# scvae/scvae

Hardware: AMD Instinct MI355X
Metric: cells/sec training (68k-PBMC NB-VAE) (higher is better)
Workload: dtype f32 (bf16x9-exact heads); 1 GPU; 68k-PBMC-shaped synthetic counts 68579x32738 (~5% nonzero, device CSR), negative binomial VAE hidden 100-100 latent 25 batch-norm, Adam lr 1e-4; global_batch=4096, parallelism=dp1

## Files before the change

scvae_amd/csrc/decoder_fused3.hip:

```cpp
#include <type_traits>

#include "common.hpp"
#include "kernels.hpp"
#include "likelihood.hpp"

namespace scvae {

typedef float f32x16 __attribute__((ext_vector_type(16)));
typedef float f32x4m __attribute__((ext_vector_type(4)));
typedef __bf16 bf16x8 __attribute__((ext_vector_type(8)));
typedef short s16x4 __attribute__((ext_vector_type(4)));
typedef short s16x8 __attribute__((ext_vector_type(8)));
typedef unsigned u32x4 __attribute__((ext_vector_type(4)));
typedef unsigned u32x2 __attribute__((ext_vector_type(2)));
typedef float f32x2 __attribute__((ext_vector_type(2)));
typedef float f32x4u __attribute__((ext_vector_type(4), aligned(4)));

#ifndef D3_PIN_LOADS
#define D3_PIN_LOADS 1
#endif
#ifndef D3_AHEAD
#define D3_AHEAD 1
#endif
constexpr int D3_NB = D3_AHEAD + 1;
__device__ __forceinline__ void d3_pin_loads() {
  if (D3_PIN_LOADS) __builtin_amdgcn_sched_barrier(0x7C6);
}

constexpr int D3_THREADS = 512;
constexpr int D3_BM = 64;
constexpr int D3_KP = 128;
__host__ __device__ constexpr int d3_bn(int P) { return P >= 3 ? 32 : 64; }
__host__ __device__ constexpr int d3_rowb(int P) { return 2 * d3_bn(P) + 16; }

__host__ __device__ inline int d3_hp1(int H) { return (H + 1 + 15) / 16 * 16; }

int decoder_fused3_strip_genes(int P) { return d3_bn(P); }
size_t decoder_fused3_lds_bytes(int P, int H) {
  return (size_t)P * 3 * d3_hp1(H) * d3_rowb(P) + (size_t)P * 3 * D3_BM * d3_rowb(P) +
         2 * D3_BM * sizeof(float);
}
bool decoder_fused3_supported(int P, int H) {
  return P <= 3 && H >= 2 && H <= 126 && decoder_fused3_lds_bytes(P, H) <= 160 * 1024;
}
__host__ __device__ inline int d3_kp(int H) { return H + 1 <= D3_KP ? D3_KP : (H + 1 + 31) / 32 * 32; }
__host__ __device__ inline size_t d3_set_elems(int Rpad, int KP = D3_KP) {
  return (size_t)2 * 3 * Rpad * KP;
}
size_t decoder_fused3_workspace_floats(int rows, int H) {
  const size_t rpad = (size_t)(rows + D3_BM - 1) / D3_BM * D3_BM;
  const int kp = d3_kp(H);
  if (kp > D3_KP) return d3_set_elems((int)rpad, kp) * sizeof(uint16_t) / sizeof(float) + 64;
  return 3 * d3_set_elems((int)rpad) * sizeof(uint16_t) / sizeof(float) + 3 * rpad * 4 + 64;
}

typedef __bf16 bf16x2 __attribute__((ext_vector_type(2)));
typedef float f32x2v __attribute__((ext_vector_type(2)));
__device__ __forceinline__ unsigned cvt_pk_bf16(float lo, float hi) {
  return __builtin_bit_cast(unsigned, __builtin_convertvector(f32x2v{lo, hi}, bf16x2));
}
__device__ __forceinline__ void split3_rn(float x, unsigned& b1, unsigned& b2, unsigned& b3) {
  b1 = cvt_pk_bf16(0.f, x) & 0xFFFF0000u;
  const float r1 = x - __uint_as_float(b1);
  b2 = cvt_pk_bf16(0.f, r1) & 0xFFFF0000u;
  b3 = __float_as_uint(r1 - __uint_as_float(b2));
}
__device__ __forceinline__ unsigned pack_hi16(unsigned lo, unsigned hi) {
  return __builtin_amdgcn_perm(hi, lo, 0x07060302u);
}
__device__ __forceinline__ void split3_rn_pair(float x0, float x1, unsigned& p1, unsigned& p2,
                                               unsigned& p3) {
  p1 = cvt_pk_bf16(x0, x1);
  float r0 = x0 - __uint_as_float(p1 << 16), r1 = x1 - __uint_as_float(p1 & 0xFFFF0000u);
  p2 = cvt_pk_bf16(r0, r1);
  r0 -= __uint_as_float(p2 << 16);
  r1 -= __uint_as_float(p2 & 0xFFFF0000u);
  p3 = pack_hi16(__float_as_uint(r0), __float_as_uint(r1));
}

__global__ __launch_bounds__(256) void split3_hidden_kernel(const float* __restrict__ d, int R,
                                                            int H, int Rpad, int KP,
                                                            uint16_t* __restrict__ dA,
                                                            uint16_t* __restrict__ dT,
                                                            u32x4* __restrict__ zero,
                                                            size_t zero16) {
  const int slot = blockIdx.x * 256 + threadIdx.x;
  for (size_t i = (size_t)(blockIdx.y * gridDim.x + blockIdx.x) * 256 + threadIdx.x; i < zero16;
       i += (size_t)gridDim.x * gridDim.y * 256)
    zero[i] = u32x4{0u, 0u, 0u, 0u};
  if (slot >= Rpad * (KP / 8)) return;
  const int ksp = KP / 32;
  const int lane = slot & 63, frag = slot >> 6;
  const int nb = Rpad / 16;
  unsigned t1[8], t2[8], t3[8];
  auto value = [&](int r, int k) {
    if (r >= R) return 0.f;
    return k < H ? d[(size_t)r * H + k] : (k == H ? 1.f : 0.f);
  };
  if (blockIdx.y == 0) {
    const int rb = frag / ksp, ks = frag % ksp;
    const int row = 16 * rb + (lane & 15), k0 = 32 * ks + 8 * (lane >> 4);
#pragma unroll
    for (int e = 0; e < 8; ++e) split3_rn(value(row, k0 + e), t1[e], t2[e], t3[e]);
  } else {
    const int ht = frag / nb, kg = frag % nb;
    const int h = 32 * ht + (lane & 31), r0 = 16 * kg + 8 * (lane >> 5);
#pragma unroll
    for (int e = 0; e < 8; ++e) split3_rn(value(r0 + e, h), t1[e], t2[e], t3[e]);
  }
  auto pack = [](const unsigned* t) {
    u32x4 v;
    v.x = pack_hi16(t[0], t[1]); v.y = pack_hi16(t[2], t[3]);
    v.z = pack_hi16(t[4], t[5]); v.w = pack_hi16(t[6], t[7]);
    return v;
  };
  const size_t plane = (size_t)KP * Rpad;
  uint16_t* dst = (blockIdx.y == 0 ? dA : dT) + (size_t)slot * 8;
  *reinterpret_cast<u32x4*>(dst) = pack(t1);
  *reinterpret_cast<u32x4*>(dst + plane) = pack(t2);
  *reinterpret_cast<u32x4*>(dst + 2 * plane) = pack(t3);
}

__device__ __forceinline__ bf16x8 lds_b128(const char* p) {
  return __builtin_bit_cast(bf16x8, *reinterpret_cast<const u32x4*>(p));
}
__device__ __forceinline__ s16x4 lds_tr(const char* p) {
  return __builtin_amdgcn_ds_read_tr16_b64_v4i16(
      (__attribute__((address_space(3))) s16x4*)(p));
}
template <int ROWB>
__device__ __forceinline__ bf16x8 lds_tr8(const char* p) {
  const s16x4 lo = lds_tr(p), hi = lds_tr(p + 4 * ROWB);
  return __builtin_bit_cast(bf16x8, __builtin_shufflevector(lo, hi, 0, 1, 2, 3, 4, 5, 6, 7));
}
__device__ __forceinline__ bf16x8 global_b128(const uint16_t* p) {
  return __builtin_bit_cast(bf16x8, *reinterpret_cast<const u32x4*>(p));
}

struct IndexMasks3 { unsigned long long m[3]; };
__device__ __forceinline__ IndexMasks3 index_masks3(int idx) {
  IndexMasks3 k;
#pragma unroll
  for (int b = 0; b < 3; ++b) k.m[b] = __builtin_amdgcn_ballot_w64((idx >> b) & 1);
  return k;
}
__device__ __forceinline__ float cnd3(float lo, float hi, unsigned long long mask) {
  float r;
  asm("v_cndmask_b32_e64 %0, %1, %2, %3" : "=v"(r) : "v"(lo), "v"(hi), "s"(mask));
  return r;
}
__device__ __forceinline__ float select_n(const float (&v)[8], const IndexMasks3& k) {
  float a[4], b[2];
#pragma unroll
  for (int i = 0; i < 4; ++i) a[i] = cnd3(v[2 * i], v[2 * i + 1], k.m[0]);
#pragma unroll
  for (int i = 0; i < 2; ++i) b[i] = cnd3(a[2 * i], a[2 * i + 1], k.m[1]);
  return cnd3(b[0], b[1], k.m[2]);
}
__device__ __forceinline__ float select_n(const float (&v)[4], const IndexMasks3& k) {
  return cnd3(cnd3(v[0], v[1], k.m[0]), cnd3(v[2], v[3], k.m[0]), k.m[1]);
}

template <int KIND, int KS1, bool U16, bool TRAIN, bool DROP, int CP>
__global__ __launch_bounds__(D3_THREADS) void decoder_head3_kernel(
    const uint16_t* __restrict__ dA, const uint16_t* __restrict__ dT, int R, int Rpad, int H,
    HeadParams hp, int F, Targets tg, int B, const float* __restrict__ gw, int inline_lgamma,
    float* __restrict__ ll_part, float* __restrict__ dd_part,
    const uint32_t* __restrict__ drop_bits, float inv_keep, CpRows cp) {
  constexpr bool IDX = false;
  const int64_t* const trows = nullptr;
#include "decoder_head3_body.inc"
}
template <int KIND, int KS1, bool TRAIN>
__global__ __launch_bounds__(D3_THREADS) void decoder_head3_rows_kernel(
    const uint16_t* __restrict__ dA, const uint16_t* __restrict__ dT, int R, int Rpad, int H,
    HeadParams hp, int F, Targets tg, int B, const float* __restrict__ gw, int inline_lgamma,
    float* __restrict__ ll_part, float* __restrict__ dd_part,
    const int64_t* __restrict__ trows) {
  constexpr bool U16 = true, DROP = false, IDX = true;
  constexpr int CP = 0;
  const uint32_t* const drop_bits = nullptr;
  const float inv_keep = 1.f;
  const CpRows cp = CpRows();
#include "decoder_head3_body.inc"
}


constexpr int D4_BM = 32;

#ifndef D4_COMPACT
#define D4_COMPACT 1
#endif
__host__ __device__ constexpr bool d4_compact(int ks1) { return D4_COMPACT && ks1 <= 4; }
__host__ __device__ constexpr int d4_threads(int npw) { return (npw + 4) * 64; }
size_t decoder_fused4_lds_bytes(int P, int H, int npw, int bn = 0) {
  const int rowb = 2 * (bn ? bn : d3_bn(P)) + 16;
  return (size_t)P * 3 * d3_hp1(H) * rowb + (size_t)2 * P * 3 * D4_BM * rowb +
         (size_t)2 * (npw / 2) * 4 * D4_BM * sizeof(float) +
         (d4_compact((H + 1 + 31) / 32) ? npw * 512 : 0);
}

#ifndef D4_PROF
#define D4_PROF 0
#endif
#ifndef D4_PRIO_PRODUCER
#define D4_PRIO_PRODUCER 1
#endif
#ifndef D4_PRIO_CONSUMER
#define D4_PRIO_CONSUMER 0
#endif
#if D4_PROF
__device__ unsigned long long d4_prof[12 * 8];
#define D4_STAMP(k)                                            \
  do {                                                         \
    __builtin_amdgcn_sched_barrier(0);                         \
    const unsigned long long t_ = __builtin_amdgcn_s_memtime(); \
    pacc[k] += t_ - plast;                                     \
    plast = t_;                                                \
    __builtin_amdgcn_sched_barrier(0);                         \
  } while (0)
#define D4_PROF_BEGIN unsigned long long pacc[8] = {0, 0, 0, 0, 0, 0, 0, 0}, plast = __builtin_amdgcn_s_memtime()
#define D4_PROF_END                                                                  \
  do {                                                                               \
    if (blockIdx.x == 0 && lane == 0)                                                \
      for (int k_ = 0; k_ < 8; ++k_) d4_prof[w * 8 + k_] = pacc[k_];                 \
  } while (0)
#else
#define D4_STAMP(k) do {} while (0)
#define D4_PROF_BEGIN do {} while (0)
#define D4_PROF_END do {} while (0)
#endif

#ifndef D4_G1_EIGHT
#define D4_G1_EIGHT 0
#endif
template <int KIND, int KS1, bool U16, int NPW, int BN_ = 0, bool DBP = false,
          int G1 = (NPW == 4 ? 1 : D4_G1_EIGHT), int TERMS = 9, bool FWD = false>
__global__ __launch_bounds__(d4_threads(NPW)) void decoder_head4_kernel(
    const uint16_t* __restrict__ dA, const uint16_t* __restrict__ dT, int R, int Rpad, int H,
    HeadParams hp, int F, Targets tg, int B, const float* __restrict__ gw, int inline_lgamma,
    float* __restrict__ ll_part, float* __restrict__ dd_part, int dd_atomic, int rg_tiles,
    float* __restrict__ rg_slab) {
  constexpr bool IDX = false;
  const int64_t* const trows = nullptr;
#include "decoder_head4_body.inc"
}
template <int KIND, int KS1, int NPW, int BN_, bool DBP, int G1, bool FWD>
__global__ __launch_bounds__(d4_threads(NPW)) void decoder_head4_rows_kernel(
    const uint16_t* __restrict__ dA, const uint16_t* __restrict__ dT, int R, int Rpad, int H,
    HeadParams hp, int F, Targets tg, int B, const float* __restrict__ gw, int inline_lgamma,
    float* __restrict__ ll_part, float* __restrict__ dd_part, int dd_atomic, int rg_tiles,
    float* __restrict__ rg_slab, const int64_t* __restrict__ trows) {
  constexpr bool U16 = true, IDX = true;
  constexpr int TERMS = 9;
#include "decoder_head4_body.inc"
}

#if D4_PROF
extern "C" int scvae_d4_prof_dump(unsigned long long* out) {
  return (int)hipMemcpyFromSymbol(out, HIP_SYMBOL(d4_prof), sizeof(unsigned long long) * 96);
}
#endif

static int d3_schedule_env() {
  static const int v = [] {
    const char* e = getenv("SCVAE_D3_SCHEDULE");
    return (e && (e[0] == '3' || e[0] == '4')) ? e[0] - '0' : 0;
  }();
  return v;
}
static int d4_producers_env() {
  static const int v = [] {
    const char* e = getenv("SCVAE_D4_PRODUCERS");
    return (e && (e[0] == '4' || e[0] == '8')) ? e[0] - '0' : 0;
  }();
  return v;
}
struct D4Config { int bn, npw, ks1; size_t lds; bool ok; bool dbp; };
static D4Config d4_config(int P, int H) {
  D4Config c;
  c.ks1 = (H + 1 + 31) / 32;
  c.bn = d3_bn(P);
  c.npw = P >= 3 ? 4 : (d4_producers_env() ? d4_producers_env() : (P == 1 ? 4 : 8));
  c.lds = decoder_fused4_lds_bytes(P, H, c.npw, c.bn);
  if (c.lds > 160 * 1024 && c.bn == 64 && P == 2) {
    c.bn = 32; c.npw = 4;
    c.lds = decoder_fused4_lds_bytes(P, H, c.npw, c.bn);
  }
  if (c.ks1 > 4 && c.npw == 8) {
    c.npw = 4;
    c.lds = decoder_fused4_lds_bytes(P, H, c.npw, c.bn);
  }
  c.dbp = H >= 128 && H % 32 == 0;
  c.ok = P >= 1 && P <= 3 && H >= 2 && c.ks1 <= (c.dbp ? 9 : 8) && c.lds <= 160 * 1024;
  return c;
}
bool decoder_fused4_supported(int P, int H) { return d4_config(P, H).ok; }
static int d3_schedule(int P, int H, int rows) {
  if (!decoder_fused3_supported(P, H)) return 4;
  if (!decoder_fused4_supported(P, H)) return 3;
  return d3_schedule_env() ? d3_schedule_env() : (rows <= 128 ? 3 : 4);
}
int d4_strip_genes(int P, int H) { return d4_config(P, H).bn; }
int decoder_fused3_train_strip_genes(int P, int H, int rows, bool drop, int cp_pass) {
  if (!drop && cp_pass == 0 && d3_schedule(P, H, rows) == 4) return d4_config(P, H).bn;
  return d3_bn(P);
}

bool decoder_fused3_dd_atomics(int kind, int H, int rows, bool drop, int cp_pass, int dd_mode) {
  const int P = likelihood_heads(kind);
  return (dd_mode & 1) && !(dd_mode & 4) && !drop && cp_pass == 0 && d3_schedule(P, H, rows) == 4;
}

int decoder_fused3_train_kernel_name(int kind, int H, int rows, bool u16, char* out, size_t n,
                                     int terms) {
  const int P = likelihood_heads(kind);
  if (d3_schedule(P, H, rows) == 4) {
    const D4Config c = d4_config(P, H);
    const bool six = terms == 6 && c.ks1 <= 4 && c.bn == d3_bn(P) && !c.dbp;
    return snprintf(out, n, "decoder_head4_kernel<%d, %d, %s, %d, %d, %s, %d, %d, false>", kind, c.ks1,
                    u16 ? "true" : "false", c.npw, c.bn == d3_bn(P) ? 0 : c.bn,
                    c.dbp ? "true" : "false", c.npw == 4 ? 1 : D4_G1_EIGHT, six ? 6 : 9);
  }
  return snprintf(out, n, "decoder_head3_kernel<%d, %d, %s, true, false, 0>", kind,
                  (d3_hp1(H) + 31) / 32, u16 ? "true" : "false");
}

constexpr int D4_MAX_ROW_GROUPS = 4;
size_t decoder_fused3_rg_slab_floats(int H, int F) {
  return (size_t)(D4_MAX_ROW_GROUPS - 1) * 3 * (size_t)(H + 1) * F + 64;
}
static int d4_cu_count() {
  static thread_local int cached_device = -1, cached = 0;
  int device = 0;
  if (hipGetDevice(&device) != hipSuccess) return 256;
  if (device != cached_device) {
    hipDeviceProp_t prop;
    cached = hipGetDeviceProperties(&prop, device) == hipSuccess ? prop.multiProcessorCount : 256;
    cached_device = device;
  }
  return cached > 0 ? cached : 256;
}
static int d4_row_groups(int strips, int rows) {
  static const int forced = [] {
    const char* e = getenv("SCVAE_D4_ROW_GROUPS");
    return e ? atoi(e) : 0;
  }();
  const int tiles = (rows + D4_BM - 1) / D4_BM;
  int most = tiles / 8;
  if (most > D4_MAX_ROW_GROUPS) most = D4_MAX_ROW_GROUPS;
  if (most < 1) most = 1;
  if (forced >= 1) return forced < most ? forced : most;
  const int cus = d4_cu_count();
  int best = 1;
  double best_score = 0.0;
  for (int n = 1; n <= most; ++n) {
    const long wgs = (long)strips * n;
    const long rounds = (wgs + cus - 1) / cus;
    const double score = (double)wgs / (double)(rounds * cus) - 0.04 * (n - 1);
    if (score > best_score + 1e-9) { best = n; best_score = score; }
  }
  return best;
}
__global__ __launch_bounds__(256) void d4_rg_combine_kernel(HeadParams hp, int P, int H, int F,
                                                            const float* __restrict__ slab,
                                                            int groups) {
  const int jh = blockIdx.y;
  const int j = jh / (H + 1), h = jh % (H + 1);
  float* dst = h < H ? hp.dW[j] + (size_t)h * F : hp.db[j];
  const size_t gstride = (size_t)P * (H + 1) * F;
  const float* src = slab + ((size_t)j * (H + 1) + h) * F;
  for (int c = blockIdx.x * blockDim.x + threadIdx.x; c < F; c += gridDim.x * blockDim.x) {
    float v = dst[c];
    for (int g = 0; g < groups; ++g) v += src[(size_t)g * gstride + c];
    dst[c] = v;
  }
}

struct D4Launch {
  hipStream_t s; const uint16_t* dA; const uint16_t* dT; int rows, Rpad, H; HeadParams hp; int F;
  Targets t; int B; const float* gw; int inline_lgamma; float* ll_part; float* dd_part;
  int dd_atomic; int strips; size_t lds; int terms; int row_groups; float* rg_slab;
  bool fwd = false;
  const int64_t* trows = nullptr;
};
template <int KIND, int KS1, int NPW, int BN_, bool DBP = false, int TERMS = 9>
static int d4_launch_one(const D4Launch& a) {
  constexpr int G1 = NPW == 4 ? 1 : D4_G1_EIGHT;
  if constexpr (TERMS == 9 && KS1 <= 4 && BN_ == 0 && !DBP) {
    if (a.terms == 6) return d4_launch_one<KIND, KS1, NPW, BN_, DBP, 6>(a);
  }
  const int tiles = (a.rows + D4_BM - 1) / D4_BM;
  const int rg_tiles = (tiles + a.row_groups - 1) / a.row_groups;
  const int groups = (tiles + rg_tiles - 1) / rg_tiles;
  if (a.trows) {
    if constexpr (TERMS == 9) {
      if (!a.t.u16 || a.terms != 9) {
        set_error("decoder_head4_kernel: a row index goes with uint16 targets and nine terms");
        return -1;
      }
      auto rfn = a.fwd ? decoder_head4_rows_kernel<KIND, KS1, NPW, BN_, DBP, G1, true>
                       : decoder_head4_rows_kernel<KIND, KS1, NPW, BN_, DBP, G1, false>;
      SCVAE_HIP(max_dynamic_lds(reinterpret_cast<const void*>(rfn), (int)a.lds));
      hipLaunchKernelGGL(rfn, dim3(a.strips, groups), dim3(d4_threads(NPW)), a.lds, a.s, a.dA,
                         a.dT, a.rows, a.Rpad, a.H, a.hp, a.F, a.t, a.B, a.gw, a.inline_lgamma,
                         a.ll_part, a.dd_part, a.fwd ? 0 : a.dd_atomic, rg_tiles,
                         a.fwd ? nullptr : a.rg_slab, a.trows);
      if (!a.fwd && groups > 1) {
        constexpr int P = likelihood_heads(KIND);
        hipLaunchKernelGGL(d4_rg_combine_kernel, dim3((a.F + 1023) / 1024, P * (a.H + 1)),
                           dim3(256), 0, a.s, a.hp, P, a.H, a.F, a.rg_slab, groups - 1);
      }
      return 0;
    }
  }
  if constexpr (TERMS == 9) {
    if (a.fwd) {
      auto ffn = a.t.u16 ? decoder_head4_kernel<KIND, KS1, true, NPW, BN_, DBP, G1, 9, true>
                         : decoder_head4_kernel<KIND, KS1, false, NPW, BN_, DBP, G1, 9, true>;
      SCVAE_HIP(max_dynamic_lds(reinterpret_cast<const void*>(ffn), (int)a.lds));
      hipLaunchKernelGGL(ffn, dim3(a.strips, groups), dim3(d4_threads(NPW)), a.lds, a.s, a.dA,
                         a.dT, a.rows, a.Rpad, a.H, a.hp, a.F, a.t, a.B, a.gw, a.inline_lgamma,
                         a.ll_part, a.dd_part, 0, rg_tiles, nullptr);
      return 0;
    }
  }
  auto kfn = a.t.u16 ? decoder_head4_kernel<KIND, KS1, true, NPW, BN_, DBP, G1, TERMS>
                     : decoder_head4_kernel<KIND, KS1, false, NPW, BN_, DBP, G1, TERMS>;
  SCVAE_HIP(max_dynamic_lds(reinterpret_cast<const void*>(kfn), (int)a.lds));
  hipLaunchKernelGGL(kfn, dim3(a.strips, groups), dim3(d4_threads(NPW)), a.lds, a.s, a.dA, a.dT,
                     a.rows, a.Rpad, a.H, a.hp, a.F, a.t, a.B, a.gw, a.inline_lgamma, a.ll_part,
                     a.dd_part, a.dd_atomic, rg_tiles, a.rg_slab);
  if (groups > 1) {
    constexpr int P = likelihood_heads(KIND);
    hipLaunchKernelGGL(d4_rg_combine_kernel, dim3((a.F + 1023) / 1024, P * (a.H + 1)), dim3(256), 0,
                       a.s, a.hp, P, a.H, a.F, a.rg_slab, groups - 1);
  }
  return 0;
}
template <int KIND, int KS1>
static int d4_launch_steps(const D4Launch& a, const D4Config& c) {
  constexpr int P = likelihood_heads(KIND);
  if constexpr (KS1 >= 5) {
    if (c.dbp) {
      if constexpr (P == 1) return d4_launch_one<KIND, KS1, 4, 0, true>(a);
      else if constexpr (P == 2) return d4_launch_one<KIND, KS1, 4, 32, true>(a);
      else if constexpr (KS1 == 5) return d4_launch_one<KIND, KS1, 4, 0, true>(a);
    }
  }
  if constexpr (KS1 == 9) {
    set_error("decoder_head4_kernel: nine contraction steps only at H = 256");
    return -1;
  } else if constexpr (P == 1) {
    if constexpr (KS1 <= 4) { if (c.npw == 8) return d4_launch_one<KIND, KS1, 8, 0>(a); }
    return d4_launch_one<KIND, KS1, 4, 0>(a);
  } else if constexpr (P == 2) {
    if constexpr (KS1 <= 4) {
      if (c.bn == 64) return c.npw == 8 ? d4_launch_one<KIND, KS1, 8, 0>(a)
                                        : d4_launch_one<KIND, KS1, 4, 0>(a);
    }
    if constexpr (KS1 >= 4) return d4_launch_one<KIND, KS1, 4, 32>(a);
    set_error("decoder_head4_kernel: no instantiation for %d steps on %d-gene strips", KS1, c.bn);
    return -1;
  } else {
    if constexpr (KS1 <= 5) return d4_launch_one<KIND, KS1, 4, 0>(a);
    set_error("decoder_head4_kernel: three heads beyond H = 159");
    return -1;
  }
}
template <int KIND>
static int d4_launch_kind(const D4Launch& a, const D4Config& c) {
  switch (c.ks1) {
    case 1: return d4_launch_steps<KIND, 1>(a, c);
    case 2: return d4_launch_steps<KIND, 2>(a, c);
    case 3: return d4_launch_steps<KIND, 3>(a, c);
    case 4: return d4_launch_steps<KIND, 4>(a, c);
    case 5: return d4_launch_steps<KIND, 5>(a, c);
    case 6: return d4_launch_steps<KIND, 6>(a, c);
    case 7: return d4_launch_steps<KIND, 7>(a, c);
    case 8: return d4_launch_steps<KIND, 8>(a, c);
    case 9: return d4_launch_steps<KIND, 9>(a, c);
    default: set_error("decoder_head4_kernel: %d contraction steps", c.ks1); return -1;
  }
}

int decoder_fused3_launch(hipStream_t s, bool train, int kind, const float* d, int rows, int H,
                          HeadParams hp, int F, Targets t, int B, const float* gw,
                          int inline_lgamma, float* ll_part, float* dd_part, float* planes,
                          const HeadDropout* drop, int cp_pass, const CpRows* cp, int dd_mode,
                          float* rg_slab, const int64_t* t_rows) {
  const int P = likelihood_heads(kind);
  SCVAE_ARG(!t_rows || (t.u16 && kind <= LK_ZINB && !drop && cp_pass == 0 && !(dd_mode & 6)));
  const bool wide = !decoder_fused3_supported(P, H) ||
                    (!train && cp_pass == 0 &&
                     (P > 2 || !decoder_fused_supported(H) || (dd_mode & 8)));
  SCVAE_ARG(!(dd_mode & 4) || (train && !wide && !drop && cp_pass == 0));
  SCVAE_ARG((hp.gene_stride == 0 && t.shift == 0.f) || (dd_mode & 4));
  SCVAE_ARG(planes && (!wide || (!drop && cp_pass == 0 && decoder_fused4_supported(P, H))));
  SCVAE_ARG(train || !drop);
  SCVAE_ARG((kind == LK_CPOISSON) == (cp_pass >= 1 && cp_pass <= 3 && cp && cp->count_sum));
  SCVAE_ARG(cp_pass == 0 || ((cp_pass == 3) == train && !drop));
  const CpRows cpr = cp ? *cp : CpRows();
  const int Rpad = (rows + D3_BM - 1) / D3_BM * D3_BM;
  const int KP = d3_kp(H);
  uint16_t* dA = reinterpret_cast<uint16_t*>(planes);
  uint16_t* dT = dA + (size_t)3 * Rpad * KP;
  uint32_t* bits = reinterpret_cast<uint32_t*>(dA + 3 * d3_set_elems(Rpad));
  const bool head4_train = train && !(dd_mode & 4) && !drop && cp_pass == 0 &&
                           d3_schedule(P, H, rows) == 4;
  const size_t acc_bytes = (size_t)8 * H * rows * sizeof(float);
  const bool clear_here = head4_train && (dd_mode & 1) && (acc_bytes & 15) == 0 &&
                          (reinterpret_cast<uintptr_t>(dd_part) & 15) == 0;
  for (int j = 0; j < (drop ? P : 1); ++j) {
    hipLaunchKernelGGL(split3_hidden_kernel, dim3((Rpad * (KP / 8) + 255) / 256, train ? 2 : 1),
                       dim3(256), 0, s, drop ? drop->d[j] : d, rows, H, Rpad, KP,
                       dA + j * d3_set_elems(Rpad), dT + j * d3_set_elems(Rpad),
                       clear_here ? reinterpret_cast<u32x4*>(dd_part) : nullptr,
                       clear_here ? acc_bytes / 16 : (size_t)0);
    SCVAE_LAUNCH_CHECK("split3_hidden_kernel");
    if (drop) {
      const int rc = dropout_mask_words(s, bits + (size_t)j * Rpad * 4, rows, Rpad, H, drop->keep,
                                        drop->seed, drop->site[j], drop->map);
      if (rc) return rc;
    }
  }
  const float inv_keep = drop ? 1.f / drop->keep : 1.f;
  const size_t lds = decoder_fused3_lds_bytes(P, H);
  const int strips = (F + d3_bn(P) - 1) / d3_bn(P);
  const int ks1 = (d3_hp1(H) + 31) / 32;
#define SCVAE_D3KC(K_, KS_, T_, D_, C_)                                                          \
  do {                                                                                            \
    auto kfn = t.u16 ? decoder_head3_kernel<K_, KS_, true, T_, D_, C_>                            \
                     : decoder_head3_kernel<K_, KS_, false, T_, D_, C_>;                          \
    SCVAE_HIP(max_dynamic_lds(reinterpret_cast<const void*>(kfn), \
                                  (int)lds));         \
    hipLaunchKernelGGL(kfn, dim3(strips), dim3(D3_THREADS), lds, s, dA, dT, rows, Rpad, H, hp, F, \
                       t, B, gw, inline_lgamma, ll_part, dd_part, bits, inv_keep, cpr);           \
  } while (0)
#define SCVAE_D3K(K_, KS_, T_, D_) SCVAE_D3KC(K_, KS_, T_, D_, 0)
#define SCVAE_D3RK(K_, KS_, T_)                                                                   \
  do {                                                                                            \
    auto kfn = decoder_head3_rows_kernel<K_, KS_, T_>;                                            \
    SCVAE_HIP(max_dynamic_lds(reinterpret_cast<const void*>(kfn), (int)lds));                     \
    hipLaunchKernelGGL(kfn, dim3(strips), dim3(D3_THREADS), lds, s, dA, dT, rows, Rpad, H, hp, F, \
                       t, B, gw, inline_lgamma, ll_part, dd_part, t_rows);                        \
  } while (0)
#define SCVAE_D3R(K_, T_)                                                                         \
  switch (ks1) {                                                                                  \
    case 1: SCVAE_D3RK(K_, 1, T_); break;                                                         \
    case 2: SCVAE_D3RK(K_, 2, T_); break;                                                         \
    case 3: SCVAE_D3RK(K_, 3, T_); break;                                                         \
    default: SCVAE_D3RK(K_, 4, T_); break;                                                        \
  }
#define SCVAE_D3C(T_, C_)                                                                         \
  switch (ks1) {                                                                                  \
    case 1: SCVAE_D3KC(LK_CPOISSON, 1, T_, false, C_); break;                                     \
    case 2: SCVAE_D3KC(LK_CPOISSON, 2, T_, false, C_); break;                                     \
    case 3: SCVAE_D3KC(LK_CPOISSON, 3, T_, false, C_); break;                                     \
    default: SCVAE_D3KC(LK_CPOISSON, 4, T_, false, C_); break;                                    \
  }
#define SCVAE_D3(K_, T_, D_)                                                                      \
  switch (ks1) {                                                                                  \
    case 1: SCVAE_D3K(K_, 1, T_, D_); break;                                                      \
    case 2: SCVAE_D3K(K_, 2, T_, D_); break;                                                      \
    case 3: SCVAE_D3K(K_, 3, T_, D_); break;                                                      \
    default: SCVAE_D3K(K_, 4, T_, D_); break;                                                     \
  }
  if (train && decoder_fused_probe(0)) SCVAE_HIP(hipEventRecord(decoder_fused_probe(0), s));
  if (cp_pass == 1) {
    SCVAE_D3C(false, 1);
  } else if (cp_pass == 2) {
    SCVAE_D3C(false, 2);
  } else if (cp_pass == 3) {
    SCVAE_D3C(true, 3);
  } else if (train && drop) {
    switch (kind) {
      case LK_POISSON: SCVAE_D3(LK_POISSON, true, true); break;
      case LK_NB: SCVAE_D3(LK_NB, true, true); break;
      case LK_ZIP: SCVAE_D3(LK_ZIP, true, true); break;
      case LK_ZINB: SCVAE_D3(LK_ZINB, true, true); break;
      case LK_BERNOULLI: SCVAE_D3(LK_BERNOULLI, true, true); break;
      default: set_error("decoder_head3_kernel: likelihood kind %d", kind); return -1;
    }
  } else if ((train && !(dd_mode & 4) && d3_schedule(P, H, rows) == 4) || (!train && wide)) {
    const D4Config c = d4_config(P, H);
    D4Launch a{s, dA, dT, rows, Rpad, H, hp, F, t, B, gw, inline_lgamma, ll_part, dd_part,
               (dd_mode & 1) ? 1 : 0, (F + c.bn - 1) / c.bn, c.lds, (dd_mode & 2) ? 6 : 9, 1,
               rg_slab};
    a.fwd = !train;
    a.trows = t_rows;
    if (a.fwd) { a.dd_atomic = 0; a.terms = 9; }
    if (rg_slab || a.fwd) a.row_groups = d4_row_groups(a.strips, rows);
    if (a.dd_atomic && !clear_here)
      SCVAE_HIP(hipMemsetAsync(dd_part, 0, (size_t)8 * H * rows * sizeof(float), s));
    int rc;
    switch (kind) {
      case LK_POISSON: rc = d4_launch_kind<LK_POISSON>(a, c); break;
      case LK_NB: rc = d4_launch_kind<LK_NB>(a, c); break;
      case LK_ZIP: rc = d4_launch_kind<LK_ZIP>(a, c); break;
      case LK_ZINB: rc = d4_launch_kind<LK_ZINB>(a, c); break;
      case LK_BERNOULLI: rc = d4_launch_kind<LK_BERNOULLI>(a, c); break;
      default: set_error("decoder_head4_kernel: likelihood kind %d", kind); return -1;
    }
    if (rc) return rc;
  } else if (t_rows && train) {
    switch (kind) {
      case LK_POISSON: SCVAE_D3R(LK_POISSON, true); break;
      case LK_NB: SCVAE_D3R(LK_NB, true); break;
      case LK_ZIP: SCVAE_D3R(LK_ZIP, true); break;
      default: SCVAE_D3R(LK_ZINB, true); break;
    }
  } else if (t_rows) {
    switch (kind) {
      case LK_POISSON: SCVAE_D3R(LK_POISSON, false); break;
      case LK_NB: SCVAE_D3R(LK_NB, false); break;
      case LK_ZIP: SCVAE_D3R(LK_ZIP, false); break;
      default: set_error("decoder_head3_kernel (forward): likelihood kind %d", kind); return -1;
    }
  } else if (train) {
    switch (kind) {
      case LK_POISSON: SCVAE_D3(LK_POISSON, true, false); break;
      case LK_NB: SCVAE_D3(LK_NB, true, false); break;
      case LK_ZIP: SCVAE_D3(LK_ZIP, true, false); break;
      case LK_ZINB: SCVAE_D3(LK_ZINB, true, false); break;
      case LK_BERNOULLI: SCVAE_D3(LK_BERNOULLI, true, false); break;
      case LK_CAT2: SCVAE_D3(LK_CAT2, true, false); break;
      case LK_CAT3: SCVAE_D3(LK_CAT3, true, false); break;
      default: set_error("decoder_head3_kernel: likelihood kind %d", kind); return -1;
    }
  } else {
    switch (kind) {
      case LK_POISSON: SCVAE_D3(LK_POISSON, false, false); break;
      case LK_NB: SCVAE_D3(LK_NB, false, false); break;
      case LK_ZIP: SCVAE_D3(LK_ZIP, false, false); break;
      case LK_BERNOULLI: SCVAE_D3(LK_BERNOULLI, false, false); break;
      default: set_error("decoder_head3_kernel (forward): likelihood kind %d", kind); return -1;
    }
  }
#undef SCVAE_D3
#undef SCVAE_D3R
#undef SCVAE_D3RK
#undef SCVAE_D3C
#undef SCVAE_D3KC
#undef SCVAE_D3K
  SCVAE_LAUNCH_CHECK("decoder_head3_kernel");
  if (train && decoder_fused_probe(1)) SCVAE_HIP(hipEventRecord(decoder_fused_probe(1), s));
  return 0;
}

}
```

scvae_amd/csrc/decoder_head4_body.inc:

```
  using Traits = LikelihoodTraits<KIND>;
  constexpr int P = Traits::P;
  constexpr int NT = d4_threads(NPW);
  constexpr int BN = BN_ ? BN_ : d3_bn(P), ROWB = 2 * BN + 16;
  constexpr int NT2 = DBP ? KS1 - 1 : KS1;
  constexpr int NHT = (NT2 + 3) / 4;
  static_assert(!DBP || (NPW == 4 && KS1 >= 2), "DBP: four producers");
  constexpr int DF = KS1 < 4 ? KS1 : 4;
  constexpr int GPLANE = D4_BM * ROWB;
  constexpr int GBUF = P * 3 * GPLANE;
  constexpr int NGP = NPW / 2;
  constexpr int NSB = BN / (16 * NGP);
  static_assert(NSB >= 1 && NSB * 16 * NGP == BN, "producer waves tile the strip");
  constexpr int NE = 4 * NSB;
  constexpr int KS3 = BN / 16;
  constexpr int NGT = BN / 32;
  constexpr int LLN = NGP * 4 * D4_BM;
  extern __shared__ __attribute__((aligned(16))) char smem[];
  const int HP1 = d3_hp1(H);
  const int WPLANE = HP1 * ROWB;
  char* Wl = smem;
  char* Gl = smem + (size_t)P * 3 * WPLANE;
  float* llbuf = reinterpret_cast<float*>(Gl + 2 * GBUF);
  const int tid = threadIdx.x, lane = tid & 63;
  const int w = __builtin_amdgcn_readfirstlane(tid >> 6);
  const int q = lane >> 4, i16 = lane & 15, li = lane & 31, kh = lane >> 5;
  const int c0 = blockIdx.x * BN;
  const int dbg = D4_PROF ? inline_lgamma >> 8 : 0;
  inline_lgamma &= 0xFF;

  constexpr int HSTEP = NT / BN;
  constexpr int NV = (32 * KS1 + HSTEP - 1) / HSTEP;
  {
    const int g = tid & (BN - 1), h0 = tid / BN;
    const bool col_ok = c0 + g < F;
    const int gc = min(c0 + g, F - 1);
    float v[P][NV];
#pragma unroll
    for (int j = 0; j < P; ++j) {
      const float* wj = hp.W[j] + gc;
      const float* bj = hp.b[j] + gc;
#pragma unroll
      for (int u = 0; u < NV; ++u) {
        const int h = min(h0 + u * HSTEP, H);
        const float* src = h < H ? wj + (size_t)h * F : bj;
        v[j][u] = *src;
      }
    }
    {
      const int n16 = (int)(((size_t)P * 3 * WPLANE + 2 * GBUF + 2 * LLN * 4) / 16);
      u32x4* z = reinterpret_cast<u32x4*>(smem);
      for (int i = tid; i < n16; i += NT) z[i] = u32x4{0u, 0u, 0u, 0u};
    }
    __syncthreads();
#pragma unroll
    for (int j = 0; j < P; ++j)
#pragma unroll
      for (int u = 0; u < NV; ++u) {
        const int h = h0 + u * HSTEP;
        if (h <= H) {
          unsigned b1, b2, b3;
          split3_rn(col_ok ? v[j][u] : 0.f, b1, b2, b3);
          char* dst = Wl + (size_t)(j * 3) * WPLANE + h * ROWB + 2 * g;
          *reinterpret_cast<uint16_t*>(dst) = (uint16_t)(b1 >> 16);
          *reinterpret_cast<uint16_t*>(dst + WPLANE) = (uint16_t)(b2 >> 16);
          *reinterpret_cast<uint16_t*>(dst + 2 * WPLANE) = (uint16_t)(b3 >> 16);
        }
      }
  }
  __syncthreads();

  const int tile0 = blockIdx.y * rg_tiles;
  const int n_tiles = min((R + D4_BM - 1) / D4_BM, tile0 + rg_tiles);
  const int mfirst = tile0 * D4_BM;
  auto grad_row = [&](int j, int h) -> float* {
    if (blockIdx.y == 0) return h < H ? hp.dW[j] + (size_t)h * F : hp.db[j];
    return rg_slab + (((size_t)(blockIdx.y - 1) * P + j) * (H + 1) + h) * F;
  };
  const int KP = d3_kp(H), ksp = KP / 32;
  const size_t dplane = (size_t)Rpad * KP;
  const int nb16 = Rpad / 16;

  if (w < NPW) {
    __builtin_amdgcn_s_setprio(D4_PRIO_PRODUCER);
    const int gp = w % NGP, rq = w / NGP;
    const int gbase = 16 * NSB * gp;
    const int trw = (8 * q + (i16 >> 2)) * ROWB + 2 * (gbase + 4 * (i16 & 3));
    const int gst = (16 * rq + i16) * ROWB + 2 * (gbase + 4 * q);
    struct TileIn { f32x4m t[NSB]; float up0; };
    size_t tidx = 0;
    auto load_i = [&](int m0) -> size_t {
      const int rc = min(m0 + 16 * rq + i16, R - 1);
      return (size_t)trows[R == B ? rc : rc % B];
    };
    if (IDX) tidx = load_i(mfirst);
    auto load_t = [&](int m0) {
      TileIn in;
      const int row = m0 + 16 * rq + i16;
      const bool rok = row < R;
      in.up0 = (rok && !FWD) ? gw[row] : 0.f;
      const int rc = rok ? row : R - 1;
      const int cell = R == B ? rc : rc % B;
      const size_t trow = (IDX ? tidx : (size_t)cell) * tg.ld;
#pragma unroll
      for (int sb = 0; sb < NSB; ++sb) {
        const int c = c0 + gbase + 16 * sb + 4 * q;
        f32x4m v = {0.f, 0.f, 0.f, 0.f};
        if (U16) {
          const uint16_t* tp = static_cast<const uint16_t*>(tg.p) + trow + c;
          const u32x2 u = *reinterpret_cast<const u32x2*>(tp);
          v.x = __uint_as_float(u.x); v.y = __uint_as_float(u.y);
        } else {
          const float* tp = static_cast<const float*>(tg.p) + trow + c;
          if (c + 3 < F) {
            const f32x4u u = *reinterpret_cast<const f32x4u*>(tp);
            v.x = u.x; v.y = u.y; v.z = u.z; v.w = u.w;
          } else {
            v.x = (c < F) ? tp[0] : 0.f;
            v.y = (c + 1 < F) ? tp[1] : 0.f;
            v.z = (c + 2 < F) ? tp[2] : 0.f;
          }
        }
        in.t[sb] = v;
      }
      return in;
    };
    bf16x8 dfr[DF][3];
    auto load_dk = [&](int m0, int ks, bf16x8 (&dst)[3]) {
      const uint16_t* dbase = dA + ((size_t)(m0 / 16 + rq) * ksp + ks) * 512 + lane * 8;
#pragma unroll
      for (int pl = 0; pl < 3; ++pl) dst[pl] = global_b128(dbase + pl * dplane);
    };
    auto load_d = [&](int m0) {
#pragma unroll
      for (int ks = 0; ks < DF; ++ks) load_dk(m0, ks, dfr[ks]);
    };
    f32x4m acc1[P][NSB];
    auto gemm1 = [&](int mt) {
#pragma unroll
      for (int j = 0; j < P; ++j)
#pragma unroll
        for (int sb = 0; sb < NSB; ++sb) acc1[j][sb] = f32x4m{0.f, 0.f, 0.f, 0.f};
      bf16x8 afr[2][P][NSB][3];
      auto load_w = [&](int ks, bf16x8 (&dst)[P][NSB][3]) {
#pragma unroll
        for (int j = 0; j < P; ++j)
#pragma unroll
          for (int sb = 0; sb < NSB; ++sb)
#pragma unroll
            for (int pl = 0; pl < 3; ++pl)
              dst[j][sb][pl] = lds_tr8<ROWB>(Wl + (size_t)(j * 3 + pl) * WPLANE + trw + 32 * sb +
                                             32 * ks * ROWB);
      };
      load_w(0, afr[0]);
#pragma unroll
      for (int ks = 0; ks < KS1; ++ks) {
        if (ks + 1 < KS1) load_w(ks + 1, afr[(ks + 1) & 1]);
#pragma unroll
        for (int a = 2; a >= 0; --a)
#pragma unroll
          for (int b = 2; b >= 0; --b)
#pragma unroll
            for (int j = 0; j < P; ++j)
#pragma unroll
              for (int sb = 0; sb < NSB; ++sb)
                if (TERMS == 9 || a + b < 3) acc1[j][sb] = __builtin_amdgcn_mfma_f32_16x16x32_bf16(
                    afr[ks & 1][j][sb][a], dfr[ks % DF][b], acc1[j][sb], 0, 0, 0);
        if (ks + DF < KS1) {
          load_dk(mt, ks + DF, dfr[ks % DF]);
          d3_pin_loads();
        }
      }
    };
    float dbacc[P][NE];
#pragma unroll
    for (int j = 0; j < P; ++j)
#pragma unroll
      for (int e = 0; e < NE; ++e) dbacc[j][e] = 0.f;
    TileIn nxt = load_t(mfirst);
    if (IDX) tidx = load_i(min(mfirst + D4_BM, Rpad - D4_BM));
    load_d(mfirst);
    const bool g1last = G1 == 1 || (G1 == 2 && w >= NPW / 2);
    if (g1last) {
      gemm1(mfirst);
      load_d(min(mfirst + D4_BM, Rpad - D4_BM));
      d3_pin_loads();
    }
    D4_PROF_BEGIN;
    for (int tile = tile0; tile < n_tiles; ++tile) {
      const int m0 = tile * D4_BM;
      if (dbg & 2) { lds_barrier(); continue; }
      const TileIn cur = nxt;
      const float up = cur.up0;
      char* Gb = Gl + ((tile - tile0) & 1) * GBUF;
      float* lb = llbuf + ((tile - tile0) & 1) * LLN;
      if (!g1last) gemm1(m0);
      {
        nxt = load_t(min(m0 + D4_BM, Rpad - D4_BM));
        if (IDX) tidx = load_i(min(m0 + 2 * D4_BM, Rpad - D4_BM));
        if (!g1last) load_d(min(m0 + D4_BM, Rpad - D4_BM));
        d3_pin_loads();
      }
      float G[P][NE], tval[NE];
      float lsum = 0.f;
      unsigned nz = 0;
#pragma unroll
      for (int sb = 0; sb < NSB; ++sb) {
        if (U16) {
          const unsigned v0 = __float_as_uint(cur.t[sb][0]), v1 = __float_as_uint(cur.t[sb][1]);
          tval[4 * sb] = (float)(v0 & 0xFFFFu); tval[4 * sb + 1] = (float)(v0 >> 16);
          tval[4 * sb + 2] = (float)(v1 & 0xFFFFu); tval[4 * sb + 3] = (float)(v1 >> 16);
        } else {
#pragma unroll
          for (int e = 0; e < 4; ++e) tval[4 * sb + e] = cur.t[sb][e];
        }
#pragma unroll
        for (int e = 0; e < 4; ++e) {
          float a[P], g[P], lp, r, rgate;
#pragma unroll
          for (int j = 0; j < P; ++j) a[j] = acc1[j][sb][e];
          lik_dense<KIND, true>(tval[4 * sb + e], a, lp, g, r, rgate);
          const bool ok = c0 + gbase + 16 * sb + 4 * q + e < F;
          lsum += ok ? lp : 0.f;
#pragma unroll
          for (int j = 0; j < P; ++j) G[j][4 * sb + e] = up * g[j];
          nz |= (ok && tval[4 * sb + e] > 0.f) ? (1u << (4 * sb + e)) : 0u;
        }
      }
      D4_STAMP(1);
      if constexpr (d4_compact(KS1)) {
      if ((Traits::HAS_R || inline_lgamma) && !(dbg & 4)) {
        int pos[NE];
        int total = 0;
#pragma unroll
        for (int e = 0; e < NE; ++e) {
          const unsigned long long bal = __builtin_amdgcn_ballot_w64(((nz >> e) & 1u) != 0u);
          pos[e] = total + (int)__builtin_amdgcn_mbcnt_hi(
                               (unsigned)(bal >> 32), __builtin_amdgcn_mbcnt_lo((unsigned)bal, 0u));
          total += __builtin_popcountll(bal);
        }
        char* qb = reinterpret_cast<char*>(llbuf + 2 * LLN) + w * 512;
        auto qaddr = [&](int k) { return qb + 8 * k; };
        for (int q0 = 0; q0 < total; q0 += 64) {
#pragma unroll
          for (int e = 0; e < NE; ++e) {
            const int k = pos[e] - q0;
            if (((nz >> e) & 1u) && (unsigned)k < 64u) {
              const float lrv = Traits::HAS_R ? acc1[P - 1][e >> 2][e & 3] : 0.f;
              *reinterpret_cast<f32x2*>(qaddr(k)) = f32x2{tval[e], lrv};
            }
          }
          __builtin_amdgcn_wave_barrier();
          const bool on = lane < total - q0;
          f32x2 in = *reinterpret_cast<const f32x2*>(qaddr(lane));
          const float tt = on ? in.x : 1.f;
          float corr = 0.f, rd = 0.f;
          if (Traits::HAS_R) {
            const float lrv = on ? in.y : 0.f;
            const float r = __expf(fminf(fmaxf(lrv, -10.f), 10.f));
            const float rgate = (lrv >= -10.f && lrv <= 10.f) ? 1.f : 0.f;
            const bool small = tt <= 8.f && (U16 || tt == __builtin_rintf(tt));
            float A, D;
            if (__builtin_amdgcn_ballot_w64(!small) == 0)
              lgamma_digamma_diff_small_wave<true>(r, tt, A, D);
            else
              lgamma_digamma_diff_general<true>(r, tt, A, D);
            corr = A;
            rd = rgate * r * D;
          }
          if (inline_lgamma) corr -= lgamma1p(tt);
          if (on) *reinterpret_cast<f32x2*>(qaddr(lane)) = f32x2{corr, rd};
          __builtin_amdgcn_wave_barrier();
#pragma unroll
          for (int e = 0; e < NE; ++e) {
            const int k = pos[e] - q0;
            if (((nz >> e) & 1u) && (unsigned)k < 64u) {
              const f32x2 o = *reinterpret_cast<const f32x2*>(qaddr(k));
              lsum += o.x;
              if (Traits::HAS_R) G[P - 1][e] = fmaf(up, o.y, G[P - 1][e]);
            }
          }
          __builtin_amdgcn_wave_barrier();
        }
      }
      } else {
      if ((Traits::HAS_R || inline_lgamma) && !(dbg & 4)) {
        float lr[NE];
        if (Traits::HAS_R) {
#pragma unroll
          for (int i = 0; i < NE; ++i) lr[i] = acc1[P - 1][i >> 2][i & 3];
        }
        while (__builtin_amdgcn_ballot_w64(nz != 0) != 0) {
          const bool on = nz != 0;
          const int idx = on ? __builtin_ctz(nz) : 0;
          nz &= nz - 1;
          const IndexMasks3 km = index_masks3(idx);
          const float tt = select_n(tval, km);
          float corr = 0.f;
          if (Traits::HAS_R) {
            const float lrv = select_n(lr, km);
            const float r = __expf(fminf(fmaxf(lrv, -10.f), 10.f));
            const float rgate = (lrv >= -10.f && lrv <= 10.f) ? 1.f : 0.f;
            const bool small = !on || (tt <= 8.f && tt == __builtin_rintf(tt));
            float A, D;
            if (__builtin_amdgcn_ballot_w64(!small) == 0)
              lgamma_digamma_diff_small_wave<true>(r, on ? tt : 0.f, A, D);
            else
              lgamma_digamma_diff_general<true>(r, on ? tt : 1.f, A, D);
            corr = A;
            const float delta = on ? up * rgate * r * D : 0.f;
#pragma unroll
            for (int e = 0; e < NE; ++e) G[P - 1][e] += (idx == e) ? delta : 0.f;
          }
          if (inline_lgamma) corr -= lgamma1p(tt);
          lsum += on ? corr : 0.f;
        }
      }
      }
      D4_STAMP(2);
      if (DBP && !FWD) {
#pragma unroll
        for (int j = 0; j < P; ++j)
#pragma unroll
          for (int e = 0; e < NE; ++e) dbacc[j][e] += G[j][e];
// ... 242 lines not shown
```

Before: 2.194 million cells/s.

## Pack the sparse last contraction step of decoder head GEMM into one MFMA pass

When the hidden width plus bias leaves eight or fewer live columns in the final 32-wide K step, the split kernel writes a packed tail fragment that holds the three bf16 planes of those columns side by side. The head kernel then finishes that step with three MFMAs per output tile instead of nine, using rotated LDS weight addressing. This cuts the padded-zero MFMA work and the D-fragment loads on the last step, at the cost of an extra workspace region, a new template variant and more complex indexing. It can be switched off with SCVAE_D4_LIVE_WIDTH=0.

```diff
diff --git a/scvae_amd/csrc/decoder_fused3.hip b/scvae_amd/csrc/decoder_fused3.hip
--- a/scvae_amd/csrc/decoder_fused3.hip
+++ b/scvae_amd/csrc/decoder_fused3.hip
@@ -47,11 +47,15 @@
 __host__ __device__ inline size_t d3_set_elems(int Rpad, int KP = D3_KP) {
   return (size_t)2 * 3 * Rpad * KP;
 }
+__host__ __device__ inline size_t d3_tail_offset(int Rpad) {
+  return 3 * d3_set_elems(Rpad) + (size_t)3 * Rpad * 4 * 2;
+}
 size_t decoder_fused3_workspace_floats(int rows, int H) {
   const size_t rpad = (size_t)(rows + D3_BM - 1) / D3_BM * D3_BM;
   const int kp = d3_kp(H);
   if (kp > D3_KP) return d3_set_elems((int)rpad, kp) * sizeof(uint16_t) / sizeof(float) + 64;
-  return 3 * d3_set_elems((int)rpad) * sizeof(uint16_t) / sizeof(float) + 3 * rpad * 4 + 64;
+  return 3 * d3_set_elems((int)rpad) * sizeof(uint16_t) / sizeof(float) + 3 * rpad * 4 +
+         rpad * 16 + 64;
 }
 
 typedef __bf16 bf16x2 __attribute__((ext_vector_type(2)));
@@ -83,7 +87,8 @@
                                                             uint16_t* __restrict__ dA,
                                                             uint16_t* __restrict__ dT,
                                                             u32x4* __restrict__ zero,
-                                                            size_t zero16) {
+                                                            size_t zero16,
+                                                            uint16_t* __restrict__ dP) {
   const int slot = blockIdx.x * 256 + threadIdx.x;
   for (size_t i = (size_t)(blockIdx.y * gridDim.x + blockIdx.x) * 256 + threadIdx.x; i < zero16;
        i += (size_t)gridDim.x * gridDim.y * 256)
@@ -97,23 +102,30 @@
     if (r >= R) return 0.f;
     return k < H ? d[(size_t)r * H + k] : (k == H ? 1.f : 0.f);
   };
-  if (blockIdx.y == 0) {
-    const int rb = frag / ksp, ks = frag % ksp;
-    const int row = 16 * rb + (lane & 15), k0 = 32 * ks + 8 * (lane >> 4);
-#pragma unroll
-    for (int e = 0; e < 8; ++e) split3_rn(value(row, k0 + e), t1[e], t2[e], t3[e]);
-  } else {
-    const int ht = frag / nb, kg = frag % nb;
-    const int h = 32 * ht + (lane & 31), r0 = 16 * kg + 8 * (lane >> 5);
-#pragma unroll
-    for (int e = 0; e < 8; ++e) split3_rn(value(r0 + e, h), t1[e], t2[e], t3[e]);
-  }
   auto pack = [](const unsigned* t) {
     u32x4 v;
     v.x = pack_hi16(t[0], t[1]); v.y = pack_hi16(t[2], t[3]);
     v.z = pack_hi16(t[4], t[5]); v.w = pack_hi16(t[6], t[7]);
     return v;
   };
+  if (blockIdx.y == 0) {
+    const int rb = frag / ksp, ks = frag % ksp;
+    const int row = 16 * rb + (lane & 15), k0 = 32 * ks + 8 * (lane >> 4);
+#pragma unroll
+    for (int e = 0; e < 8; ++e) split3_rn(value(row, k0 + e), t1[e], t2[e], t3[e]);
+    if (dP && ks == H / 32 && lane < 16) {
+      u32x4* dst = reinterpret_cast<u32x4*>(dP) + (size_t)rb * 64 + lane;
+      dst[0] = pack(t1);
+      dst[16] = pack(t2);
+      dst[32] = pack(t3);
+      dst[48] = u32x4{0u, 0u, 0u, 0u};
+    }
+  } else {
+    const int ht = frag / nb, kg = frag % nb;
+    const int h = 32 * ht + (lane & 31), r0 = 16 * kg + 8 * (lane >> 5);
+#pragma unroll
+    for (int e = 0; e < 8; ++e) split3_rn(value(r0 + e, h), t1[e], t2[e], t3[e]);
+  }
   const size_t plane = (size_t)KP * Rpad;
   uint16_t* dst = (blockIdx.y == 0 ? dA : dT) + (size_t)slot * 8;
   *reinterpret_cast<u32x4*>(dst) = pack(t1);
@@ -235,7 +247,7 @@
 #define D4_G1_EIGHT 0
 #endif
 template <int KIND, int KS1, bool U16, int NPW, int BN_ = 0, bool DBP = false,
-          int G1 = (NPW == 4 ? 1 : D4_G1_EIGHT), int TERMS = 9, bool FWD = false>
+          int G1 = (NPW == 4 ? 1 : D4_G1_EIGHT), int TERMS = 9, bool FWD = false, int LW = 0>
 __global__ __launch_bounds__(d4_threads(NPW)) void decoder_head4_kernel(
     const uint16_t* __restrict__ dA, const uint16_t* __restrict__ dT, int R, int Rpad, int H,
     HeadParams hp, int F, Targets tg, int B, const float* __restrict__ gw, int inline_lgamma,
@@ -245,7 +257,7 @@
   const int64_t* const trows = nullptr;
 #include "decoder_head4_body.inc"
 }
-template <int KIND, int KS1, int NPW, int BN_, bool DBP, int G1, bool FWD>
+template <int KIND, int KS1, int NPW, int BN_, bool DBP, int G1, bool FWD, int LW = 0>
 __global__ __launch_bounds__(d4_threads(NPW)) void decoder_head4_rows_kernel(
     const uint16_t* __restrict__ dA, const uint16_t* __restrict__ dT, int R, int Rpad, int H,
     HeadParams hp, int F, Targets tg, int B, const float* __restrict__ gw, int inline_lgamma,
@@ -275,6 +287,13 @@
     return (e && (e[0] == '4' || e[0] == '8')) ? e[0] - '0' : 0;
   }();
   return v;
+}
+static int d4_live_width(int ks1, int H, bool dbp) {
+  static const int on = [] {
+    const char* e = getenv("SCVAE_D4_LIVE_WIDTH");
+    return (e && e[0] == '0') ? 0 : 1;
+  }();
+  return (on && !dbp && ks1 <= 4 && H + 1 - 32 * (ks1 - 1) <= 8) ? 1 : 0;
 }
 struct D4Config { int bn, npw, ks1; size_t lds; bool ok; bool dbp; };
 static D4Config d4_config(int P, int H) {
@@ -318,9 +337,10 @@
   if (d3_schedule(P, H, rows) == 4) {
     const D4Config c = d4_config(P, H);
     const bool six = terms == 6 && c.ks1 <= 4 && c.bn == d3_bn(P) && !c.dbp;
-    return snprintf(out, n, "decoder_head4_kernel<%d, %d, %s, %d, %d, %s, %d, %d, false>", kind, c.ks1,
-                    u16 ? "true" : "false", c.npw, c.bn == d3_bn(P) ? 0 : c.bn,
-                    c.dbp ? "true" : "false", c.npw == 4 ? 1 : D4_G1_EIGHT, six ? 6 : 9);
+    return snprintf(out, n, "decoder_head4_kernel<%d, %d, %s, %d, %d, %s, %d, %d, false, %d>", kind,
+                    c.ks1, u16 ? "true" : "false", c.npw, c.bn == d3_bn(P) ? 0 : c.bn,
+                    c.dbp ? "true" : "false", c.npw == 4 ? 1 : D4_G1_EIGHT, six ? 6 : 9,
+                    d4_live_width(c.ks1, H, c.dbp));
   }
   return snprintf(out, n, "decoder_head3_kernel<%d, %d, %s, true, false, 0>", kind,
                   (d3_hp1(H) + 31) / 32, u16 ? "true" : "false");
@@ -384,11 +404,15 @@
   bool fwd = false;
   const int64_t* trows = nullptr;
 };
-template <int KIND, int KS1, int NPW, int BN_, bool DBP = false, int TERMS = 9>
+template <int KIND, int KS1, int NPW, int BN_, bool DBP = false, int TERMS = 9, int LW = 0>
 static int d4_launch_one(const D4Launch& a) {
   constexpr int G1 = NPW == 4 ? 1 : D4_G1_EIGHT;
-  if constexpr (TERMS == 9 && KS1 <= 4 && BN_ == 0 && !DBP) {
+  if constexpr (TERMS == 9 && KS1 <= 4 && BN_ == 0 && !DBP && LW == 0) {
     if (a.terms == 6) return d4_launch_one<KIND, KS1, NPW, BN_, DBP, 6>(a);
+  }
+  if constexpr (LW == 0 && KS1 <= 4 && !DBP) {
+    if (d4_live_width(KS1, a.H, DBP) == 1)
+      return d4_launch_one<KIND, KS1, NPW, BN_, DBP, TERMS, 1>(a);
   }
   const int tiles = (a.rows + D4_BM - 1) / D4_BM;
   const int rg_tiles = (tiles + a.row_groups - 1) / a.row_groups;
@@ -399,8 +423,8 @@
         set_error("decoder_head4_kernel: a row index goes with uint16 targets and nine terms");
         return -1;
       }
-      auto rfn = a.fwd ? decoder_head4_rows_kernel<KIND, KS1, NPW, BN_, DBP, G1, true>
-                       : decoder_head4_rows_kernel<KIND, KS1, NPW, BN_, DBP, G1, false>;
+      auto rfn = a.fwd ? decoder_head4_rows_kernel<KIND, KS1, NPW, BN_, DBP, G1, true, LW>
+                       : decoder_head4_rows_kernel<KIND, KS1, NPW, BN_, DBP, G1, false, LW>;
       SCVAE_HIP(max_dynamic_lds(reinterpret_cast<const void*>(rfn), (int)a.lds));
       hipLaunchKernelGGL(rfn, dim3(a.strips, groups), dim3(d4_threads(NPW)), a.lds, a.s, a.dA,
                          a.dT, a.rows, a.Rpad, a.H, a.hp, a.F, a.t, a.B, a.gw, a.inline_lgamma,
@@ -416,8 +440,8 @@
   }
   if constexpr (TERMS == 9) {
     if (a.fwd) {
-      auto ffn = a.t.u16 ? decoder_head4_kernel<KIND, KS1, true, NPW, BN_, DBP, G1, 9, true>
-                         : decoder_head4_kernel<KIND, KS1, false, NPW, BN_, DBP, G1, 9, true>;
+      auto ffn = a.t.u16 ? decoder_head4_kernel<KIND, KS1, true, NPW, BN_, DBP, G1, 9, true, LW>
+                         : decoder_head4_kernel<KIND, KS1, false, NPW, BN_, DBP, G1, 9, true, LW>;
       SCVAE_HIP(max_dynamic_lds(reinterpret_cast<const void*>(ffn), (int)a.lds));
       hipLaunchKernelGGL(ffn, dim3(a.strips, groups), dim3(d4_threads(NPW)), a.lds, a.s, a.dA,
                          a.dT, a.rows, a.Rpad, a.H, a.hp, a.F, a.t, a.B, a.gw, a.inline_lgamma,
@@ -425,8 +449,8 @@
       return 0;
     }
   }
-  auto kfn = a.t.u16 ? decoder_head4_kernel<KIND, KS1, true, NPW, BN_, DBP, G1, TERMS>
-                     : decoder_head4_kernel<KIND, KS1, false, NPW, BN_, DBP, G1, TERMS>;
+  auto kfn = a.t.u16 ? decoder_head4_kernel<KIND, KS1, true, NPW, BN_, DBP, G1, TERMS, false, LW>
+                     : decoder_head4_kernel<KIND, KS1, false, NPW, BN_, DBP, G1, TERMS, false, LW>;
   SCVAE_HIP(max_dynamic_lds(reinterpret_cast<const void*>(kfn), (int)a.lds));
   hipLaunchKernelGGL(kfn, dim3(a.strips, groups), dim3(d4_threads(NPW)), a.lds, a.s, a.dA, a.dT,
                      a.rows, a.Rpad, a.H, a.hp, a.F, a.t, a.B, a.gw, a.inline_lgamma, a.ll_part,
@@ -511,12 +535,15 @@
   const size_t acc_bytes = (size_t)8 * H * rows * sizeof(float);
   const bool clear_here = head4_train && (dd_mode & 1) && (acc_bytes & 15) == 0 &&
                           (reinterpret_cast<uintptr_t>(dd_part) & 15) == 0;
+  const int lw = (!drop && cp_pass == 0 && KP == D3_KP && decoder_fused4_supported(P, H))
+                     ? d4_live_width((H + 1 + 31) / 32, H, false) : 0;
   for (int j = 0; j < (drop ? P : 1); ++j) {
     hipLaunchKernelGGL(split3_hidden_kernel, dim3((Rpad * (KP / 8) + 255) / 256, train ? 2 : 1),
                        dim3(256), 0, s, drop ? drop->d[j] : d, rows, H, Rpad, KP,
                        dA + j * d3_set_elems(Rpad), dT + j * d3_set_elems(Rpad),
                        clear_here ? reinterpret_cast<u32x4*>(dd_part) : nullptr,
-                       clear_here ? acc_bytes / 16 : (size_t)0);
+                       clear_here ? acc_bytes / 16 : (size_t)0,
+                       lw ? dA + d3_tail_offset(Rpad) : nullptr);
     SCVAE_LAUNCH_CHECK("split3_hidden_kernel");
     if (drop) {
       const int rc = dropout_mask_words(s, bits + (size_t)j * Rpad * 4, rows, Rpad, H, drop->keep,
diff --git a/scvae_amd/csrc/decoder_head4_body.inc b/scvae_amd/csrc/decoder_head4_body.inc
--- a/scvae_amd/csrc/decoder_head4_body.inc
+++ b/scvae_amd/csrc/decoder_head4_body.inc
@@ -5,7 +5,11 @@
   constexpr int NT2 = DBP ? KS1 - 1 : KS1;
   constexpr int NHT = (NT2 + 3) / 4;
   static_assert(!DBP || (NPW == 4 && KS1 >= 2), "DBP: four producers");
-  constexpr int DF = KS1 < 4 ? KS1 : 4;
+  constexpr bool TAILP = LW == 1;
+  static_assert(LW == 0 || LW == 1, "live width: the packed last step or none");
+  static_assert(!TAILP || (KS1 <= 4 && !DBP), "packed last step: up to four contraction steps");
+  constexpr int KSF = TAILP ? KS1 - 1 : KS1;
+  constexpr int DF = KSF < 4 ? (KSF > 0 ? KSF : 1) : 4;
   constexpr int GPLANE = D4_BM * ROWB;
   constexpr int GBUF = P * 3 * GPLANE;
   constexpr int NGP = NPW / 2;
@@ -130,10 +134,21 @@
 #pragma unroll
       for (int pl = 0; pl < 3; ++pl) dst[pl] = global_b128(dbase + pl * dplane);
     };
+    bf16x8 dtl;
+    const uint16_t* const dP = dA + d3_tail_offset(Rpad);
     auto load_d = [&](int m0) {
 #pragma unroll
-      for (int ks = 0; ks < DF; ++ks) load_dk(m0, ks, dfr[ks]);
+      for (int ks = 0; ks < DF && ks < KSF; ++ks) load_dk(m0, ks, dfr[ks]);
+      if (TAILP) dtl = global_b128(dP + ((size_t)(m0 / 16 + rq) * 64 + lane) * 8);
     };
+    int trt[3];
+#pragma unroll
+    for (int r = 0; r < 3; ++r) {
+      const int a = (q + r) % 3;
+      const bool dead = TERMS != 9 && q < 3 && a + q >= 3;
+      trt[r] = a * WPLANE + ((dead ? 8 : 0) + (i16 >> 2) + 32 * (KS1 - 1)) * ROWB +
+               2 * (gbase + 4 * (i16 & 3));
+    }
     f32x4m acc1[P][NSB];
     auto gemm1 = [&](int mt) {
 #pragma unroll
@@ -151,10 +166,21 @@
               dst[j][sb][pl] = lds_tr8<ROWB>(Wl + (size_t)(j * 3 + pl) * WPLANE + trw + 32 * sb +
                                              32 * ks * ROWB);
       };
-      load_w(0, afr[0]);
-#pragma unroll
-      for (int ks = 0; ks < KS1; ++ks) {
-        if (ks + 1 < KS1) load_w(ks + 1, afr[(ks + 1) & 1]);
+      auto load_wt = [&](bf16x8 (&dst)[P][NSB][3]) {
+#pragma unroll
+        for (int j = 0; j < P; ++j)
+#pragma unroll
+          for (int sb = 0; sb < NSB; ++sb)
+#pragma unroll
+            for (int r = 0; r < 3; ++r)
+              dst[j][sb][r] = lds_tr8<ROWB>(Wl + (size_t)(j * 3) * WPLANE + trt[r] + 32 * sb);
+      };
+      if (KSF > 0) load_w(0, afr[0]);
+      else load_wt(afr[0]);
+#pragma unroll
+      for (int ks = 0; ks < KSF; ++ks) {
+        if (ks + 1 < KSF) load_w(ks + 1, afr[(ks + 1) & 1]);
+        else if (TAILP) load_wt(afr[(ks + 1) & 1]);
 #pragma unroll
         for (int a = 2; a >= 0; --a)
 #pragma unroll
@@ -165,10 +191,20 @@
               for (int sb = 0; sb < NSB; ++sb)
                 if (TERMS == 9 || a + b < 3) acc1[j][sb] = __builtin_amdgcn_mfma_f32_16x16x32_bf16(
                     afr[ks & 1][j][sb][a], dfr[ks % DF][b], acc1[j][sb], 0, 0, 0);
-        if (ks + DF < KS1) {
+        if (ks + DF < KSF) {
           load_dk(mt, ks + DF, dfr[ks % DF]);
           d3_pin_loads();
         }
+      }
+      if (TAILP) {
+#pragma unroll
+        for (int r = 2; r >= 0; --r)
+#pragma unroll
+          for (int j = 0; j < P; ++j)
+#pragma unroll
+            for (int sb = 0; sb < NSB; ++sb)
+              acc1[j][sb] = __builtin_amdgcn_mfma_f32_16x16x32_bf16(afr[KSF & 1][j][sb][r], dtl,
+                                                                    acc1[j][sb], 0, 0, 0);
       }
     };
     float dbacc[P][NE];
```

Result: faster. 2.241 million cells/s, median of 6 (+2.2%).
